# mhpi/hydrodl2

Measured on AMD Instinct MI355X. Metric: basin-ensemble-timesteps/sec fwd+bwd, higher is better.
Workload: dtype f32

## Files before the change

__graft_entry__.py:

```python
from __future__ import annotations

import os
import subprocess
import sys

ROOT = os.path.dirname(os.path.abspath(__file__))
CSRC = os.path.join(ROOT, "hydrodl2_amd", "csrc")
HIP_LIB = os.path.join(CSRC, "libhbvx.so")
ORACLE_DIR = os.path.join(ROOT, "oracle")
ORACLE_LIB = os.path.join(ORACLE_DIR, "liboracle_hbv.so")

HIPCC_FLAGS = ["--offload-arch=gfx950", "-O3", "-std=c++17", "-ffp-contract=off", "-fno-slp-vectorize", "-fPIC"]


def _newer(target: str, *sources: str) -> bool:
    if not os.path.exists(target):
        return False
    t = os.path.getmtime(target)
    return all(os.path.getmtime(s) <= t for s in sources)


def _hipcc() -> str:
    hipcc = os.environ.get("HIPCC", "/opt/rocm/bin/hipcc")
    return hipcc if os.path.exists(hipcc) else "hipcc"


def build_hip(force: bool = False, tag: str = "", flags=()) -> str:
    from concurrent.futures import ThreadPoolExecutor
    units = [os.path.join(CSRC, f) for f in sorted(os.listdir(CSRC)) if f.endswith(".hip")]
    headers = [os.path.join(CSRC, f) for f in sorted(os.listdir(CSRC)) if f.endswith(".h")] + [
        os.path.join(ROOT, "include", "hbvx.h"), os.path.join(ROOT, "include", "hbvx_lstm.h"),
        os.path.join(ROOT, "include", "hbvx_gage_pop.h")]
    objdir = os.path.join(CSRC, "build_" + tag if tag else "build")
    os.makedirs(objdir, exist_ok=True)
    extra = os.environ.get("HBVX_EXTRA_HIPCC_FLAGS", "").split() + list(flags)
    lib = os.path.join(CSRC, f"libhbvx_{tag}.so") if tag else HIP_LIB

    def compile_one(src):
        obj = os.path.join(objdir, os.path.basename(src)[:-4] + ".o")
        if force or not _newer(obj, src, *headers):
            subprocess.check_call([_hipcc()] + HIPCC_FLAGS + extra + ["-c", src, "-o", obj], cwd=CSRC)
            return obj, True
        return obj, False

    with ThreadPoolExecutor(max_workers=min(len(units), os.cpu_count() or 1)) as pool:
        done = list(pool.map(compile_one, units))
    objs = [o for o, _ in done]
    if force or any(r for _, r in done) or not _newer(lib, *objs):
        subprocess.check_call([_hipcc(), "--offload-arch=gfx950", "-shared", "-fPIC", "-o", lib] + objs, cwd=CSRC)
    return lib


def build_oracle() -> str:
    subprocess.check_call(["make", "-C", ORACLE_DIR], stdout=subprocess.DEVNULL)
    return ORACLE_LIB
# ... 57 lines not shown
```

hydrodl2_amd/_abi.py:

```python
from __future__ import annotations

import ctypes as C
import os
from typing import NamedTuple, Optional

ABI_VERSION = 10
MAX_PARAM = 20
GAGE_MAXLEN = 72
NSTATE = 5
MAX_FLUX = 12
UH_MAXLEN = 15

MODEL_HBV10, MODEL_HBV11P, MODEL_HBV20, MODEL_HBVADJ, MODEL_HOURLY = 0, 1, 2, 3, 4

TRAJ_ROWS, TRAJ_PACKED, TRAJ_CKPT = 0, 1, 2

(F_QSIM, F_Q0, F_Q1, F_Q2, F_AET, F_SWE, F_RECHARGE, F_EXCS, F_EVAPFACTOR, F_TOSOIL, F_PERC,
 F_CAPILLARY) = range(12)

PARAM_SLOTS = ["parBETA", "parFC", "parK0", "parK1", "parK2", "parLP", "parPERC", "parUZL",
               "parTT", "parCFMAX", "parCFR", "parCWH", "parBETAET", "parC", "parRT", "parAC",
               "parF0", "parFMIN", "parALPHA"]

_fp = C.c_void_p
# ... 211 lines not shown
GAGE_POP_ABI_VERSION = 1


class PopRunoff(C.Structure):
    _fields_ = [("abi_version", C.c_int32), ("n_cand", C.c_int32), ("p", PopSrc * MAX_PARAM), ("runoff", _fp)]


class GagePop(C.Structure):
    _fields_ = [("abi_version", C.c_int32), ("n_cand", C.c_int32), ("runoff", _fp), ("runoff_c_stride", C.c_int64),
                ("dp", _fp), ("uh", _fp), ("transform", C.c_int32), ("n_periods", C.c_int32),
                ("period_end", C.c_void_p),
                ("target", _fp), ("w", _fp), ("shift", _fp), ("eps", _fp),
                ("sse", _fp), ("s1", _fp), ("s2", _fp), ("s3", _fp), ("sim", _fp), ("series", _fp)]


GAGE_POP_SIGNATURES = [
    ("hbvx_gage_pop_sizeof", False, _u64, [_int], None),
    ("hbvx_hourly_population_runoff", False, _int, [_P(Desc), _P(PopRunoff), _vp], (0, PopRunoff)),
    ("hbvx_gage_population_workspace_bytes", False, _u64, [_P(GageDesc), _P(GagePop)], (1, GagePop)),
    ("hbvx_gage_population_stats", False, _int, [_P(GageDesc), _P(GagePop), _vp, _u64, _vp], (1, GagePop)),
]


class HbvxError(RuntimeError):
    pass


class Library:

    def __init__(self, path: str):
        if not os.path.exists(path):
            raise FileNotFoundError(path)
        self.path = path
        self.dll = C.CDLL(path)
        d = self.dll
        for name in EXPORTS:
            if not hasattr(d, name):
                raise HbvxError(f"{path}: missing export {name}")
        self.missing = [name for name in OPTIONAL_EXPORTS + [row[0] for row in GAGE_POP_SIGNATURES] if not hasattr(d, name)]
        checked = set()
        for name, _, restype, argtypes, layout, sizeof in [row + ("hbvx_sizeof",) for row in SIGNATURES] + \
                [row + ("hbvx_gage_pop_sizeof",) for row in GAGE_POP_SIGNATURES]:
            if name in self.missing:
                continue
            fn = getattr(d, name)
            fn.restype, fn.argtypes = restype, argtypes
            if layout is not None and (sizeof, layout[0]) not in checked and sizeof not in self.missing:
                checked.add((sizeof, layout[0]))
                which, st = layout
                got = getattr(d, sizeof)(which)
                if got != C.sizeof(st):
                    raise HbvxError(f"{path}: layout mismatch for {st.__name__}: {got} != {C.sizeof(st)}")
        if d.hbvx_version() != ABI_VERSION:
            raise HbvxError(f"{path}: ABI version {d.hbvx_version()} != {ABI_VERSION}")
        for which, st in enumerate([Desc, FwdOut, BwdIO, RouteDesc, ParamSrc, ParamGrad, GageDesc]):
            if d.hbvx_sizeof(which) != C.sizeof(st):
                raise HbvxError(f"{path}: layout mismatch for {st.__name__}: "
                                f"{d.hbvx_sizeof(which)} != {C.sizeof(st)}")
        self.backend = d.hbvx_backend().decode()
        self.saves_pow = "+savepow" in self.backend

    @property
    def is_device(self) -> bool:
        return self.backend.startswith("hip")

# ... 190 lines not shown
                                                        None if gp is None else C.byref(gp), ws, C.c_uint64(ws_bytes),
                                                        C.c_void_p(stream)), "hbvx_gage_population_stats")

    def lstm_check(self, r: LstmDesc, ws, stream: int):
        self._check(self.dll.hbvx_lstm_check(C.byref(r), ws, C.c_void_p(stream)), "hbvx_lstm_check")

    def bfi(self, T: int, B: int, qs: int, q2: int, nearzero: float, out: int, stream: int):
        self._check(self.dll.hbvx_bfi(T, B, qs, q2, C.c_float(nearzero), out, C.c_void_p(stream)),
                    "hbvx_bfi")

    def route_forward(self, r: RouteDesc, q: int, uh: int, q_rout: int, stream: int):
        self._check(self.dll.hbvx_route_forward(C.byref(r), q, uh, q_rout, C.c_void_p(stream)),
                    "hbvx_route_forward")

    def route_workspace_bytes(self, r: RouteDesc) -> int:
        return int(self.dll.hbvx_route_workspace_bytes(C.byref(r)))

    def route_backward(self, r: RouteDesc, q: int, uh: int, gqr: int, gq: int, gra, grb,
                       ws, ws_bytes: int, stream: int):
        self._check(self.dll.hbvx_route_backward(C.byref(r), q, uh, gqr, gq, gra, grb, ws,
                                                 C.c_uint64(ws_bytes), C.c_void_p(stream)),
                    "hbvx_route_backward")


def _population_method(entry: str):
    def call(self, desc, args, stream: int):
        self.require(entry)
        self._check(getattr(self.dll, entry)(None if desc is None else C.byref(desc),
                                             None if args is None else C.byref(args), C.c_void_p(stream)), entry)
    call.__name__ = entry[len("hbvx_"):]
    call.__doc__ = (f"{entry}; `desc` / `args` (its {POPULATION[entry].struct.__name__}) may be None (the ABI's own "
                    "refusals are under test).")
    return call


for _name in POPULATION:
    setattr(Library, _name[len("hbvx_"):], _population_method(_name))
```

hydrodl2_amd/csrc/hbv_chunked.h:

```cpp
#pragma once

#include <hip/hip_runtime.h>

#include "../../include/hbvx.h"
#include "hbv_step.h"
#include "hbv_lane.h"
#include "hbv_onepass_compose.h"

namespace hbvx {

struct ChunkArgs {
    hbvx_desc d;
    hbvx_bwd_io io;
    int lgMp;
    int C;
    int nchunk;
    float *phi;
    float *abnd;
    float *gpart;
    int nd;
    int dslot[3];
    int per_xcd;
    int group;
};
// ... 657 lines not shown
    const int b = (int)(n / d.M), j = (int)(n % d.M);
    if (d.raw_sigmoid) {
        const float u = sigmoid_(d.p[i].sta[(int64_t)b * d.p[i].sta_b_stride + j]);
        gsum = gsum * (u * (1.0f - u));
    }
    float *dst = io.g[i].sta + (int64_t)b * io.g[i].sta_b_stride + j;
    *dst += gsum;
}

#define ONEPASS_FOLD_GROUP 4
template <int NP>
__global__ void __launch_bounds__(256) k_bwd_chunk_fold(const ChunkArgs A)
{
    constexpr int NR = onepass_rows(NP);
    const hbvx_desc &d = A.d;
    const int64_t N = (int64_t)d.B * d.M;
    const int64_t n = (int64_t)blockIdx.x * 256 + threadIdx.x;
    if (n >= N) return;
    const int grp = blockIdx.y;
    const int c0 = grp * ONEPASS_FOLD_GROUP, c1 = min(A.nchunk, c0 + ONEPASS_FOLD_GROUP);
    double acc[NP];
#pragma unroll
    for (int i = 0; i < NP; i++) acc[i] = 0.0;
    for (int c = c0; c < c1; c++) {
        const float *g = A.gpart + (int64_t)c * NR * N + n;
        const float *ab = A.abnd + (int64_t)c * 5 * N + n;
        double a[5];
#pragma unroll
        for (int k = 0; k < 5; k++) a[k] = ab[(int64_t)k * N];
#pragma unroll
        for (int i = 0; i < NP; i++) {
            const int k0 = onepass_kmin(i), r0 = onepass_row(i);
            double v = g[(int64_t)(r0 + 5 - k0) * N];
#pragma unroll
            for (int k = 0; k < 5; k++)
                if (k >= k0) v += (double)g[(int64_t)(r0 + k - k0) * N] * a[k];
            acc[i] += v;
        }
    }
    float *dst = A.phi + (int64_t)grp * NP * N + n;
#pragma unroll
    for (int i = 0; i < NP; i++) dst[(int64_t)i * N] = (float)acc[i] * (d.p[i].hi - d.p[i].lo);
}

#endif

}
```

hydrodl2_amd/csrc/hbv_pop.h:

```cpp
#pragma once

#include <math.h>
#include <stdint.h>

#if defined(__HIPCC__)
#define HBVX_POP_HD __host__ __device__ __forceinline__
#else
#define HBVX_POP_HD inline
#endif

namespace hbvx_popk {

constexpr int UH = 15;

HBVX_POP_HD void gamma_taps(float a, float bb, int L, float (&w)[UH])
{
    float aa = fmaxf(a, 0.0f) + 0.1f;
    float theta = fmaxf(bb, 0.0f) + 0.5f;
    float denom = expf(lgammaf(aa)) * powf(theta, aa);
    float sum = 0.0f;
#pragma unroll
    for (int k = 0; k < UH; k++) {
        float t = (float)k + 0.5f;
        float mid = powf(t, aa - 1.0f);
        float right = expf(-t / theta);
        w[k] = (k < L) ? 1.0f / denom * mid * right : 0.0f;
        sum += w[k];
    }
#pragma unroll
    for (int k = 0; k < UH; k++) w[k] = (k < L) ? w[k] / sum : 0.0f;
}

struct Basin {
    float uh[UH], win[UH];
    float cost;
    bool routed;
// ... 418 lines not shown
```

hydrodl2_amd/csrc/hbvx.hip:

```cpp
#include "hbvx_host.h"
#include "hbv_step.h"
#include "hbv_lane.h"
#include "hbv_gage.h"

using namespace hbvx;
using namespace hbvx_host;

static thread_local char g_err[512] = "";

int hbvx_host::fail(int code, const char *msg)
{
    snprintf(g_err, sizeof g_err, "%s", msg);
    return code;
}

int hbvx_host::hip_fail(hipError_t e, const char *what)
{
    snprintf(g_err, sizeof g_err, "%s: %s", what, hipGetErrorString(e));
    return HBVX_E_DEVICE;
}

static std::mutex g_disp_mu;
static char g_disp[2][48] = {"", ""};
void hbvx_host::note_dispatch(int dir, const char *family)
{
    std::lock_guard<std::mutex> lock(g_disp_mu);
// ... 296 lines not shown
        for (int i = 0; i < NP; i++) {
            if (!io.g[i].sta) continue;
            float gr = raw ? gsta[i] * (usta[i] * (1.0f - usta[i])) : gsta[i];
            float *dst = io.g[i].sta + (int64_t)L.b * io.g[i].sta_b_stride + L.j;
            *dst += gr;
        }
        if (io.grad_state_in) {
#pragma unroll
            for (int k = 0; k < 5; k++) io.grad_state_in[k * N + L.n] = a[k];
        }
    }
}

__device__ __forceinline__ void route_ab(const hbvx_route_desc &r, int b, float &ua, float &ub,
                                         float &a, float &bb)
{
    float va = r.ra[(int64_t)b * r.r_stride], vb = r.rb[(int64_t)b * r.r_stride];
    ua = r.raw_sigmoid ? sigmoid_(va) : va;
    ub = r.raw_sigmoid ? sigmoid_(vb) : vb;
    a = descale_(ua, r.a_lo, r.a_hi);
    bb = descale_(ub, r.b_lo, r.b_hi);
}

__global__ void k_uh_gamma(const hbvx_route_desc r, float *__restrict__ uh)
{
    int b = blockIdx.x * blockDim.x + threadIdx.x;
    if (b >= r.B) return;
    float ua, ub, a, bb;
    route_ab(r, b, ua, ub, a, bb);
    float aa = fmaxf(a, 0.0f) + 0.1f;
    float theta = fmaxf(bb, 0.0f) + 0.5f;
    float denom = expf(lgammaf(aa)) * powf(theta, aa);
    float w[HBVX_UH_MAXLEN];
    float sum = 0.0f;
#pragma unroll
    for (int k = 0; k < HBVX_UH_MAXLEN; k++) {
        float t = (float)k + 0.5f;
        float mid = powf(t, aa - 1.0f);
        float right = expf(-t / theta);
        w[k] = (k < r.L) ? 1.0f / denom * mid * right : 0.0f;
        sum += w[k];
    }
#pragma unroll
    for (int k = 0; k < HBVX_UH_MAXLEN; k++)
        if (k < r.L) uh[(int64_t)b * r.L + k] = w[k] / sum;
}

#ifndef ROUTE_CHUNK
#define ROUTE_CHUNK 32
#endif
#ifndef ROUTE_CHUNK_BWD
#define ROUTE_CHUNK_BWD 64
#endif

__device__ __forceinline__ void load_uh(const float *__restrict__ uh, int b, int L, float *w)
{
#pragma unroll
    for (int k = 0; k < HBVX_UH_MAXLEN; k++) w[k] = (k < L) ? uh[(int64_t)b * L + k] : 0.0f;
}

#ifndef ROUTE_GROUP
#define ROUTE_GROUP 8
#endif
__global__ void __launch_bounds__(256) k_route_fwd(int T, int B, int S, int L,
                                                   const float *__restrict__ q,
                                                   const float *__restrict__ uh,
                                                   float *__restrict__ y)
{
    const int b = blockIdx.x * 64 + (threadIdx.x & 63);
    const int chunk = blockIdx.y * 4 + (threadIdx.x >> 6);
    const int t0 = chunk * ROUTE_CHUNK;
    if (b >= B || t0 >= T) return;
    const int t1 = min(T, t0 + ROUTE_CHUNK);
    const int s = blockIdx.z;
    float w[HBVX_UH_MAXLEN];
    load_uh(uh, b, L, w);
    const float *qs = q + (int64_t)s * T * B + b;
    float *ys = y + (int64_t)s * T * B + b;
    float win[HBVX_UH_MAXLEN];
#pragma unroll
    for (int k = 1; k < HBVX_UH_MAXLEN; k++) win[k] = (t0 - k >= 0) ? qs[(int64_t)(t0 - k) * B] : 0.0f;
    for (int tg = t0; tg < t1; tg += ROUTE_GROUP) {
        float v[ROUTE_GROUP];
#pragma unroll
        for (int j = 0; j < ROUTE_GROUP; j++) v[j] = (tg + j < t1) ? qs[(int64_t)(tg + j) * B] : 0.0f;
#pragma unroll
        for (int j = 0; j < ROUTE_GROUP; j++) {
            win[0] = v[j];
            float acc = 0.0f;
#pragma unroll
            for (int k = 0; k < HBVX_UH_MAXLEN; k++) acc += w[k] * win[k];
            if (tg + j < t1) ys[(int64_t)(tg + j) * B] = acc;
#pragma unroll
            for (int k = HBVX_UH_MAXLEN - 1; k > 0; k--) win[k] = win[k - 1];
        }
    }
}

__global__ void __launch_bounds__(256) k_route_bwd(int T, int B, int S, int L,
                                                   const float *__restrict__ q,
                                                   const float *__restrict__ uh,
                                                   const float *__restrict__ gy,
                                                   float *__restrict__ gq, double *__restrict__ ws)
{
    const int b = blockIdx.x * 64 + (threadIdx.x & 63);
    const int chunk = blockIdx.y * 4 + (threadIdx.x >> 6);
    const int t0 = chunk * ROUTE_CHUNK_BWD;
    if (b >= B || t0 >= T) return;
    const int t1 = min(T, t0 + ROUTE_CHUNK_BWD);
    float w[HBVX_UH_MAXLEN];
    double gw[HBVX_UH_MAXLEN];
    load_uh(uh, b, L, w);
#pragma unroll
    for (int k = 0; k < HBVX_UH_MAXLEN; k++) gw[k] = 0.0;
    for (int s = 0; s < S; s++) {
    const float *qs = q + (int64_t)s * T * B + b;
    const float *gs = gy + (int64_t)s * T * B + b;
    float *gqs = gq + (int64_t)s * T * B + b;
    float qwin[HBVX_UH_MAXLEN], gwin[HBVX_UH_MAXLEN];
#pragma unroll
    for (int k = 1; k < HBVX_UH_MAXLEN; k++) qwin[k] = (t0 - k >= 0) ? qs[(int64_t)(t0 - k) * B] : 0.0f;
#pragma unroll
    for (int k = 0; k < HBVX_UH_MAXLEN - 1; k++) gwin[k + 1] = (t0 + k < T) ? gs[(int64_t)(t0 + k) * B] : 0.0f;
    for (int tg = t0; tg < t1; tg += ROUTE_GROUP) {
        float vq[ROUTE_GROUP], vg[ROUTE_GROUP];
#pragma unroll
        for (int j = 0; j < ROUTE_GROUP; j++) {
            const int t = tg + j;
            vq[j] = (t < t1) ? qs[(int64_t)t * B] : 0.0f;
            vg[j] = (t + HBVX_UH_MAXLEN - 1 < T) ? gs[(int64_t)(t + HBVX_UH_MAXLEN - 1) * B] : 0.0f;
        }
#pragma unroll
        for (int j = 0; j < ROUTE_GROUP; j++) {
            const bool on = tg + j < t1;
#pragma unroll
            for (int k = 0; k < HBVX_UH_MAXLEN - 1; k++) gwin[k] = gwin[k + 1];
            gwin[HBVX_UH_MAXLEN - 1] = vg[j];
            qwin[0] = vq[j];
            float acc = 0.0f;
            const double g0 = on ? (double)gwin[0] : 0.0;
#pragma unroll
            for (int k = 0; k < HBVX_UH_MAXLEN; k++) {
                acc += w[k] * gwin[k];
                gw[k] = fma(g0, (double)qwin[k], gw[k]);
            }
            if (on) gqs[(int64_t)(tg + j) * B] = acc;
#pragma unroll
            for (int k = HBVX_UH_MAXLEN - 1; k > 0; k--) qwin[k] = qwin[k - 1];
        }
    }
    }
    if (ws) {
#pragma unroll
        for (int k = 0; k < HBVX_UH_MAXLEN; k++)
            if (k < L) ws[((int64_t)chunk * L + k) * B + b] = gw[k];
    }
}

__global__ void __launch_bounds__(256) k_route_tan_batch(const hbvx_route_desc r, const float *__restrict__ q,
                                                         const float *__restrict__ uh, const float *__restrict__ qd_all,
                                                         int64_t qd_ds, const float *__restrict__ rad_all,
                                                         const float *__restrict__ rbd_all, int64_t r_ds,
                                                         float *__restrict__ yd_all)
{
    const int T = r.T, B = r.B, L = r.L;
    const int b = blockIdx.x * 64 + (threadIdx.x & 63);
    const int chunk = blockIdx.y * 4 + (threadIdx.x >> 6);
    const int t0 = chunk * ROUTE_CHUNK;
    if (b >= B || t0 >= T) return;
    const int t1 = min(T, t0 + ROUTE_CHUNK);
    const int dir = blockIdx.z / r.S, s = blockIdx.z - dir * r.S;
    const float *qd = qd_all ? qd_all + dir * qd_ds : nullptr;
    const float *rad = rad_all ? rad_all + dir * r_ds : nullptr, *rbd = rbd_all ? rbd_all + dir * r_ds : nullptr;
    float *yd = yd_all + (int64_t)dir * r.S * T * B;
    float ua, ub, a, bb;
    route_ab(r, b, ua, ub, a, bb);
    const float theta = fmaxf(bb, 0.0f) + 0.5f;
    float dua = rad ? rad[(int64_t)b * r.r_stride] : 0.0f, dub = rbd ? rbd[(int64_t)b * r.r_stride] : 0.0f;
// ... 38 lines not shown
        for (int k = HBVX_UH_MAXLEN - 1; k > 0; k--) {
            win[k] = win[k - 1];
            dwin[k] = dwin[k - 1];
        }
    }
}

#define ROUTE_PB 16
__global__ void __launch_bounds__(1024) k_route_bwd_params(const hbvx_route_desc r, int nchunk,
                                                           const float *__restrict__ uh,
                                                           const double *__restrict__ ws,
                                                           float *grad_ra, float *grad_rb)
{
    __shared__ double prt[4][16][ROUTE_PB];
    __shared__ double red[16][ROUTE_PB];
    const int bl = threadIdx.x & (ROUTE_PB - 1), k = (threadIdx.x >> 4) & 15, part = threadIdx.x >> 8;
    const int b = blockIdx.x * ROUTE_PB + bl;
    const int B = r.B, L = r.L;
    double acc = 0.0;
    if (b < B && k < L) {
        const double *src = ws + (int64_t)k * B + b;
        const int64_t cs = (int64_t)L * B;
        const int n4 = nchunk & ~3;
        for (int c = part; c < n4; c += 4) acc += src[(int64_t)c * cs];
        if (part == 0)
            for (int c = n4; c < nchunk; c++) acc += src[(int64_t)c * cs];
    }
    prt[part][k][bl] = acc;
    __syncthreads();
    if (part == 0) red[k][bl] = (prt[0][k][bl] + prt[1][k][bl]) + (prt[2][k][bl] + prt[3][k][bl]);
    __syncthreads();
    if (part != 0 || k != 0 || b >= B) return;
    float ua, ub, a, bb;
    route_ab(r, b, ua, ub, a, bb);
    const float theta = fmaxf(bb, 0.0f) + 0.5f;
    double w[HBVX_UH_MAXLEN], gw[HBVX_UH_MAXLEN];
    double mlt = 0.0, mt = 0.0;
#pragma unroll
    for (int j = 0; j < HBVX_UH_MAXLEN; j++) {
        gw[j] = (j < L) ? red[j][bl] : 0.0;
        w[j] = (j < L) ? (double)uh[(int64_t)b * L + j] : 0.0;
        const double tk = (double)j + 0.5;
        mlt += w[j] * log(tk);
        mt += w[j] * tk;
    }
    double gaa = 0.0, gth = 0.0;
    const double th2 = (double)theta * (double)theta;
// ... 212 lines not shown
    });
    if (e != hipSuccess) return hip_fail(e, "hbvx_backward launch");
    return HBVX_OK;
}

static int check_route(const hbvx_route_desc *r)
{
    if (!r) return fail(HBVX_E_NULL, "route desc is NULL");
    if (r->abi_version != HBVX_ABI_VERSION) return fail(HBVX_E_ABI, "abi_version mismatch");
    if (r->T <= 0 || r->B <= 0 || r->S <= 0) return fail(HBVX_E_SHAPE, "bad T/B/S");
    const int L = r->T < HBVX_UH_MAXLEN ? r->T : HBVX_UH_MAXLEN;
    if (r->L != L) return fail(HBVX_E_SHAPE, "L must be min(T, 15)");
    if (!r->ra || !r->rb) return fail(HBVX_E_NULL, "routing parameter pointer is NULL");
    return HBVX_OK;
}

extern "C" int hbvx_route_forward(const hbvx_route_desc *r, const float *q, float *uh,
                                  float *q_rout, void *stream)
{
    int rc = check_route(r);
    if (rc) return rc;
    if (!q || !uh || !q_rout) return fail(HBVX_E_NULL, "route buffer is NULL");
    hipStream_t st = (hipStream_t)stream;
    hipLaunchKernelGGL(k_uh_gamma, dim3((r->B + 63) / 64), dim3(64), 0, st, *r, uh);
    const int nchunk = (r->T + ROUTE_CHUNK - 1) / ROUTE_CHUNK;
    hipLaunchKernelGGL(k_route_fwd, dim3((r->B + 63) / 64, (nchunk + 3) / 4, r->S), dim3(256), 0, st, r->T,
                       r->B, r->S, r->L, q, uh, q_rout);
    hipError_t e = hipGetLastError();
    if (e != hipSuccess) return hip_fail(e, "hbvx_route_forward launch");
    return HBVX_OK;
}

static int route_chunks(const hbvx_route_desc *r) { return (r->T + ROUTE_CHUNK_BWD - 1) / ROUTE_CHUNK_BWD; }

extern "C" uint64_t hbvx_route_workspace_bytes(const hbvx_route_desc *r)
{
    if (!r || r->T <= 0 || r->B <= 0) return 0;
    return (uint64_t)route_chunks(r) * (uint64_t)r->L * (uint64_t)r->B * sizeof(double);
}

extern "C" int hbvx_route_backward(const hbvx_route_desc *r, const float *q, const float *uh,
                                   const float *grad_q_rout, float *grad_q, float *grad_ra,
                                   float *grad_rb, void *workspace, uint64_t workspace_bytes,
                                   void *stream)
{
    int rc = check_route(r);
    if (rc) return rc;
    if (!q || !uh || !grad_q_rout || !grad_q) return fail(HBVX_E_NULL, "route buffer is NULL");
    hipStream_t st = (hipStream_t)stream;
    const bool want_p = grad_ra || grad_rb;
    if (want_p && (!workspace || workspace_bytes < hbvx_route_workspace_bytes(r)))
        return fail(HBVX_E_NULL, "route workspace missing or too small");
    const int nchunk = route_chunks(r);
    hipLaunchKernelGGL(k_route_bwd, dim3((r->B + 63) / 64, (nchunk + 3) / 4), dim3(256), 0, st, r->T,
                       r->B, r->S, r->L, q, uh, grad_q_rout, grad_q, want_p ? (double *)workspace : nullptr);
    if (want_p)
        hipLaunchKernelGGL(k_route_bwd_params, dim3((r->B + ROUTE_PB - 1) / ROUTE_PB), dim3(1024), 0, st, *r, nchunk,
                           uh, (const double *)workspace, grad_ra, grad_rb);
    hipError_t e = hipGetLastError();
    if (e != hipSuccess) return hip_fail(e, "hbvx_route_backward launch");
    return HBVX_OK;
}

__global__ void k_selftest_pow(const float *x, const float *y, float *out, int n)
{
    int i = blockIdx.x * blockDim.x + threadIdx.x;
    if (i < n) out[i] = pow_pos_(x[i], y[i]);
}

extern "C" int hbvx_selftest_pow(const float *x, const float *y, float *out, int n, void *stream)
{
    if (!x || !y || !out || n <= 0) return fail(HBVX_E_NULL, "selftest_pow: bad arguments");
    hipLaunchKernelGGL(k_selftest_pow, dim3((n + 255) / 256), dim3(256), 0, (hipStream_t)stream, x, y,
                       out, n);
    hipError_t e = hipGetLastError();
    if (e != hipSuccess) return hip_fail(e, "selftest_pow launch");
    return HBVX_OK;
}

__global__ void k_selftest_div(const float *x, const float *y, float *out, int n)
{
    int i = blockIdx.x * blockDim.x + threadIdx.x;
    if (i < n) out[i] = div_(x[i], y[i]);
}

extern "C" int hbvx_selftest_div(const float *x, const float *y, float *out, int n, void *stream)
{
    if (!x || !y || !out || n <= 0) return fail(HBVX_E_NULL, "selftest_div: bad arguments");
    hipLaunchKernelGGL(k_selftest_div, dim3((n + 255) / 256), dim3(256), 0, (hipStream_t)stream, x, y,
                       out, n);
    hipError_t e = hipGetLastError();
    if (e != hipSuccess) return hip_fail(e, "selftest_div launch");
    return HBVX_OK;
}

__global__ void __launch_bounds__(1024) k_bfi(int T, int B, const float *__restrict__ qs,
                                              const float *__restrict__ q2, float nz,
                                              float *__restrict__ bfi)
{
    __shared__ float r0[64][16], r2[64][16];
    const int bl = threadIdx.x & 15, sl = threadIdx.x >> 4;
    const int b = blockIdx.x * 16 + bl;
    float a0 = 0.0f, a2 = 0.0f, c0 = 0.0f, c2 = 0.0f;
    if (b < B) {
        int t = sl;
        for (; t + 64 < T; t += 128) {
            a0 += qs[(int64_t)t * B + b];
            a2 += q2[(int64_t)t * B + b];
            c0 += qs[(int64_t)(t + 64) * B + b];
            c2 += q2[(int64_t)(t + 64) * B + b];
        }
        if (t < T) {
            a0 += qs[(int64_t)t * B + b];
            a2 += q2[(int64_t)t * B + b];
        }
    }
    r0[sl][bl] = a0 + c0;
    r2[sl][bl] = a2 + c2;
    __syncthreads();
    if (sl == 0 && b < B) {
        float s0 = 0.0f, s2 = 0.0f;
#pragma unroll
        for (int k = 0; k < 64; k++) {
            s0 += r0[k][bl];
            s2 += r2[k][bl];
        }
        bfi[b] = 100.0f * (s2 / (s0 + nz));
    }
}

extern "C" int hbvx_bfi(int32_t T, int32_t B, const float *qs, const float *q2, float nearzero,
                        float *bfi, void *stream)
{
    if (!qs || !q2 || !bfi || T <= 0 || B <= 0) return fail(HBVX_E_NULL, "hbvx_bfi: bad arguments");
    hipLaunchKernelGGL(k_bfi, dim3((B + 15) / 16), dim3(1024), 0, (hipStream_t)stream, T, B, qs, q2,
                       nearzero, bfi);
    hipError_t e = hipGetLastError();
    if (e != hipSuccess) return hip_fail(e, "hbvx_bfi launch");
    return HBVX_OK;
}

__device__ __forceinline__ void bfi_tan_body(int T, int B, const float *__restrict__ qs,
                                             const float *__restrict__ q2, const float *__restrict__ qsd,
                                             const float *__restrict__ q2d, float nz, float *__restrict__ bfid)
{
    __shared__ float r0[64][16], r2[64][16], d0[64][16], d2[64][16];
    const int bl = threadIdx.x & 15, sl = threadIdx.x >> 4;
    const int b = blockIdx.x * 16 + bl;
    float a0 = 0.0f, a2 = 0.0f, e0 = 0.0f, e2 = 0.0f;
    if (b < B) {
        for (int t = sl; t < T; t += 64) {
            a0 += qs[(int64_t)t * B + b];
            a2 += q2[(int64_t)t * B + b];
            e0 += qsd ? qsd[(int64_t)t * B + b] : 0.0f;
            e2 += q2d ? q2d[(int64_t)t * B + b] : 0.0f;
        }
    }
    r0[sl][bl] = a0;
    r2[sl][bl] = a2;
// ... 351 lines not shown
```

hydrodl2_amd/ops.py:

```python
from __future__ import annotations

import contextlib
import ctypes as _C
from dataclasses import dataclass, field
import functools
import os
import struct
import threading
from typing import List, NamedTuple, Optional, Sequence

import torch
import torch.autograd.forward_ad as _fwAD

from . import _abi
from ._lib import get_library


@dataclass
class ParamSource:
    slot: int
    lo: float
    hi: float
    tensor_idx: int
    sta_off: int
# ... 543 lines not shown
        if _FILL_OVERLAP and lib.is_device:
            gp, rows, bases, start_fill = _overlapped_grad_buffers(lib, cfg, ptensors, ctx.needs_input_grad[6:], early)
        else:
            gp = [_grad_like(lib, p, cfg, i) if ctx.needs_input_grad[6 + i] else None
                  for i, p in enumerate(ptensors)]

        def sta_ptr(idx, off):
            return _ptr(rows[idx], off - bases[idx]) if rows[idx] is not None else _ptr(gp[idx], off)

        def join():
            nonlocal fill_done
            if start_fill is not None and fill_done is None:
                fill_done = start_fill()
            if fill_done is not None:
                torch.cuda.current_stream(dev).wait_event(fill_done)
            for big, row in zip(gp, rows):
                if row is not None:
                    big[-1] += row

        gq = None
        if g_routed is not None and cfg.route is not None:
            r = _route_desc(cfg, ptensors, S=n_live)
            gq = _out((4, T, B), dev)
            if n_live < 4:
                gq[n_live:].zero_()
            rs = cfg.route
            gt = gp[rs.tensor_idx]
            ws_bytes = _cached(cfg, ("route_ws", n_live), lambda: lib.route_workspace_bytes(r))
            ws = torch.empty((max(ws_bytes, 4) + 3) // 4, dtype=torch.float32, device=dev)
            g_routed = g_routed.contiguous()
            _call(lib, 'hbvx_route_backward', lib.route_backward, r, _ptr(flux), _ptr(uh),
                  _ptr(g_routed), _ptr(gq), sta_ptr(rs.tensor_idx, rs.a_off) if gt is not None else None,
                  sta_ptr(rs.tensor_idx, rs.b_off) if gt is not None else None,
                  _ptr(ws), ws_bytes, stream)
        have = [k for k, g in enumerate(g_rows) if g is not None]
        g_flux = None
        if have and max(have) < 4:
            if gq is None:
                gq = torch.zeros((4, T, B), dtype=torch.float32, device=dev)
            for k in have:
                gq[k] += g_rows[k]
        elif have:
            g_flux = torch.zeros((cfg.n_flux, T, B), dtype=torch.float32, device=dev)
            for k in have:
                g_flux[k] = g_rows[k]

        io = _abi.BwdIO()
        io.traj, io.aux = _ptr(traj), _ptr(aux)
        io.grad_flux, io.grad_flux4 = _ptr(g_flux), _ptr(gq)
        io.n_flux, io.traj_layout = cfg.n_flux, ctx.traj_layout
        gx = gmu = None
        if ctx.needs_input_grad[1]:
            gx = _zeros_like(lib, x)
            if gx.stride() != x.stride():
                raise ValueError("x_phy must be dense for a forcing gradient")
            io.grad_x = _ptr(gx, cfg.t0 * x.stride(0))
        if muwts is not None and ctx.needs_input_grad[3]:
# ... 861 lines not shown
```

Baseline: 34.55 billion.

## Stage routing windows in LDS, swizzle blocks across XCDs, fuse gradient zeroing

The routing forward and backward kernels now stage the q and gradient windows in shared memory and split taps and days across the four waves. Blocks are remapped so that consecutive tiles land on the same XCD. A new rows entry point zeroes the unused gq rows inside the backward launch instead of using a separate fill. Separately, the gamma unit hydrograph is computed with one thread per tap, the BFI reduction gets wider unrolled variants with XCD swizzling, and the onepass fold loads two chunks at a time. Together these aim to cut redundant global loads and launch overhead, at the cost of more shared memory per block and more code paths.

Result: faster. 35.94 billion, median of 6 (+4.0%).

```diff
diff --git a/__graft_entry__.py b/__graft_entry__.py
--- a/__graft_entry__.py
+++ b/__graft_entry__.py
@@ -30,7 +30,7 @@
     units = [os.path.join(CSRC, f) for f in sorted(os.listdir(CSRC)) if f.endswith(".hip")]
     headers = [os.path.join(CSRC, f) for f in sorted(os.listdir(CSRC)) if f.endswith(".h")] + [
         os.path.join(ROOT, "include", "hbvx.h"), os.path.join(ROOT, "include", "hbvx_lstm.h"),
-        os.path.join(ROOT, "include", "hbvx_gage_pop.h")]
+        os.path.join(ROOT, "include", "hbvx_gage_pop.h"), os.path.join(ROOT, "include", "hbvx_route_rows.h")]
     objdir = os.path.join(CSRC, "build_" + tag if tag else "build")
     os.makedirs(objdir, exist_ok=True)
     extra = os.environ.get("HBVX_EXTRA_HIPCC_FLAGS", "").split() + list(flags)
diff --git a/hydrodl2_amd/_abi.py b/hydrodl2_amd/_abi.py
--- a/hydrodl2_amd/_abi.py
+++ b/hydrodl2_amd/_abi.py
@@ -257,6 +257,11 @@
 ]
 
 
+ROUTE_ROWS_SIGNATURES = [
+    ("hbvx_route_backward_rows", False, _int, [_P(RouteDesc), _fp, _fp, _fp, _fp, _i32, _fp, _fp, _fp, _u64, _vp], None),
+]
+
+
 class HbvxError(RuntimeError):
     pass
 
@@ -272,10 +277,12 @@
         for name in EXPORTS:
             if not hasattr(d, name):
                 raise HbvxError(f"{path}: missing export {name}")
-        self.missing = [name for name in OPTIONAL_EXPORTS + [row[0] for row in GAGE_POP_SIGNATURES] if not hasattr(d, name)]
+        self.missing = [name for name in OPTIONAL_EXPORTS + [row[0] for row in GAGE_POP_SIGNATURES + ROUTE_ROWS_SIGNATURES]
+                        if not hasattr(d, name)]
         checked = set()
         for name, _, restype, argtypes, layout, sizeof in [row + ("hbvx_sizeof",) for row in SIGNATURES] + \
-                [row + ("hbvx_gage_pop_sizeof",) for row in GAGE_POP_SIGNATURES]:
+                [row + ("hbvx_gage_pop_sizeof",) for row in GAGE_POP_SIGNATURES] + \
+                [row + ("hbvx_sizeof",) for row in ROUTE_ROWS_SIGNATURES]:
             if name in self.missing:
                 continue
             fn = getattr(d, name)
@@ -512,6 +519,13 @@
                                                  C.c_uint64(ws_bytes), C.c_void_p(stream)),
                     "hbvx_route_backward")
 
+    def route_backward_rows(self, r: RouteDesc, q: int, uh: int, gqr: int, gq: int, gq_rows: int, gra, grb,
+                            ws, ws_bytes: int, stream: int):
+        self.require("hbvx_route_backward_rows")
+        self._check(self.dll.hbvx_route_backward_rows(C.byref(r), q, uh, gqr, gq, gq_rows, gra, grb, ws,
+                                                      C.c_uint64(ws_bytes), C.c_void_p(stream)),
+                    "hbvx_route_backward_rows")
+
 
 def _population_method(entry: str):
     def call(self, desc, args, stream: int):
diff --git a/hydrodl2_amd/csrc/hbv_chunked.h b/hydrodl2_amd/csrc/hbv_chunked.h
--- a/hydrodl2_amd/csrc/hbv_chunked.h
+++ b/hydrodl2_amd/csrc/hbv_chunked.h
@@ -703,21 +703,40 @@
     double acc[NP];
 #pragma unroll
     for (int i = 0; i < NP; i++) acc[i] = 0.0;
-    for (int c = c0; c < c1; c++) {
+    auto load = [&](int c, float (&gv)[NR], float (&av)[5]) {
         const float *g = A.gpart + (int64_t)c * NR * N + n;
         const float *ab = A.abnd + (int64_t)c * 5 * N + n;
+#pragma unroll
+        for (int k = 0; k < 5; k++) av[k] = ab[(int64_t)k * N];
+#pragma unroll
+        for (int r = 0; r < NR; r++) gv[r] = g[(int64_t)r * N];
+    };
+    auto fold = [&](const float (&gv)[NR], const float (&av)[5]) {
         double a[5];
 #pragma unroll
-        for (int k = 0; k < 5; k++) a[k] = ab[(int64_t)k * N];
+        for (int k = 0; k < 5; k++) a[k] = av[k];
 #pragma unroll
         for (int i = 0; i < NP; i++) {
             const int k0 = onepass_kmin(i), r0 = onepass_row(i);
-            double v = g[(int64_t)(r0 + 5 - k0) * N];
+            double v = gv[r0 + 5 - k0];
 #pragma unroll
             for (int k = 0; k < 5; k++)
-                if (k >= k0) v += (double)g[(int64_t)(r0 + k - k0) * N] * a[k];
+                if (k >= k0) v += (double)gv[r0 + k - k0] * a[k];
             acc[i] += v;
         }
+    };
+    int c = c0;
+    for (; c + 1 < c1; c += 2) {
+        float g0[NR], a0[5], g1[NR], a1[5];
+        load(c, g0, a0);
+        load(c + 1, g1, a1);
+        fold(g0, a0);
+        fold(g1, a1);
+    }
+    if (c < c1) {
+        float g0[NR], a0[5];
+        load(c, g0, a0);
+        fold(g0, a0);
     }
     float *dst = A.phi + (int64_t)grp * NP * N + n;
 #pragma unroll
diff --git a/hydrodl2_amd/csrc/hbv_pop.h b/hydrodl2_amd/csrc/hbv_pop.h
--- a/hydrodl2_amd/csrc/hbv_pop.h
+++ b/hydrodl2_amd/csrc/hbv_pop.h
@@ -12,6 +12,15 @@
 namespace hbvx_popk {
 
 constexpr int UH = 15;
+
+HBVX_POP_HD float gamma_denom(float aa, float theta) { return expf(lgammaf(aa)) * powf(theta, aa); }
+HBVX_POP_HD float gamma_tap(float denom, float aa, float theta, int k)
+{
+    float t = (float)k + 0.5f;
+    float mid = powf(t, aa - 1.0f);
+    float right = expf(-t / theta);
+    return 1.0f / denom * mid * right;
+}
 
 HBVX_POP_HD void gamma_taps(float a, float bb, int L, float (&w)[UH])
 {
diff --git a/hydrodl2_amd/csrc/hbvx.hip b/hydrodl2_amd/csrc/hbvx.hip
--- a/hydrodl2_amd/csrc/hbvx.hip
+++ b/hydrodl2_amd/csrc/hbvx.hip
@@ -1,7 +1,9 @@
 #include "hbvx_host.h"
+#include "../../include/hbvx_route_rows.h"
 #include "hbv_step.h"
 #include "hbv_lane.h"
 #include "hbv_gage.h"
+#include "hbv_pop.h"
 
 using namespace hbvx;
 using namespace hbvx_host;
@@ -344,28 +346,29 @@
     bb = descale_(ub, r.b_lo, r.b_hi);
 }
 
-__global__ void k_uh_gamma(const hbvx_route_desc r, float *__restrict__ uh)
-{
-    int b = blockIdx.x * blockDim.x + threadIdx.x;
-    if (b >= r.B) return;
-    float ua, ub, a, bb;
-    route_ab(r, b, ua, ub, a, bb);
-    float aa = fmaxf(a, 0.0f) + 0.1f;
-    float theta = fmaxf(bb, 0.0f) + 0.5f;
-    float denom = expf(lgammaf(aa)) * powf(theta, aa);
-    float w[HBVX_UH_MAXLEN];
+#define UH_PB 16
+__global__ void __launch_bounds__(16 * UH_PB) k_uh_gamma(const hbvx_route_desc r, float *__restrict__ uh)
+{
+    static_assert(HBVX_UH_MAXLEN <= 16, "k_uh_gamma: 16 tap slots");
+    __shared__ float sw[16][UH_PB];
+    const int bl = threadIdx.x % UH_PB, k = threadIdx.x / UH_PB;
+    const int b = blockIdx.x * UH_PB + bl;
+    const bool mine = b < r.B && k < r.L;
+    float v = 0.0f;
+    if (mine) {
+        float ua, ub, a, bb;
+        route_ab(r, b, ua, ub, a, bb);
+        float aa = fmaxf(a, 0.0f) + 0.1f;
+        float theta = fmaxf(bb, 0.0f) + 0.5f;
+        v = hbvx_popk::gamma_tap(hbvx_popk::gamma_denom(aa, theta), aa, theta, k);
+    }
+    sw[k][bl] = v;
+    __syncthreads();
+    if (!mine) return;
     float sum = 0.0f;
 #pragma unroll
-    for (int k = 0; k < HBVX_UH_MAXLEN; k++) {
-        float t = (float)k + 0.5f;
-        float mid = powf(t, aa - 1.0f);
-        float right = expf(-t / theta);
-        w[k] = (k < r.L) ? 1.0f / denom * mid * right : 0.0f;
-        sum += w[k];
-    }
-#pragma unroll
-    for (int k = 0; k < HBVX_UH_MAXLEN; k++)
-        if (k < r.L) uh[(int64_t)b * r.L + k] = w[k] / sum;
+    for (int j = 0; j < HBVX_UH_MAXLEN; j++) sum += sw[j][bl];
+    uh[(int64_t)b * r.L + k] = v / sum;
 }
 
 #ifndef ROUTE_CHUNK
@@ -375,107 +378,154 @@
 #define ROUTE_CHUNK_BWD 64
 #endif
 
+static inline unsigned xcd_grid(int64_t n) { return (unsigned)((n + 7) / 8 * 8); }
+__device__ __forceinline__ int xcd_block()
+{
+    const int per = gridDim.x / 8;
+    return (blockIdx.x % 8) * per + blockIdx.x / 8;
+}
+
 __device__ __forceinline__ void load_uh(const float *__restrict__ uh, int b, int L, float *w)
 {
 #pragma unroll
     for (int k = 0; k < HBVX_UH_MAXLEN; k++) w[k] = (k < L) ? uh[(int64_t)b * L + k] : 0.0f;
 }
 
-#ifndef ROUTE_GROUP
-#define ROUTE_GROUP 8
-#endif
+#define ROUTE_FWD_TILE (4 * ROUTE_CHUNK)
+#define ROUTE_FWD_ROWS (ROUTE_FWD_TILE + HBVX_UH_MAXLEN - 1)
 __global__ void __launch_bounds__(256) k_route_fwd(int T, int B, int S, int L,
                                                    const float *__restrict__ q,
                                                    const float *__restrict__ uh,
                                                    float *__restrict__ y)
 {
-    const int b = blockIdx.x * 64 + (threadIdx.x & 63);
-    const int chunk = blockIdx.y * 4 + (threadIdx.x >> 6);
-    const int t0 = chunk * ROUTE_CHUNK;
-    if (b >= B || t0 >= T) return;
-    const int t1 = min(T, t0 + ROUTE_CHUNK);
-    const int s = blockIdx.z;
+    __shared__ float sq[ROUTE_FWD_ROWS][64];
+    constexpr int NLOAD = (ROUTE_FWD_ROWS + 3) / 4;
+    const int lane = threadIdx.x & 63, part = __builtin_amdgcn_readfirstlane(threadIdx.x >> 6);
+    const int nx = (B + 63) / 64, ny = (T + ROUTE_FWD_TILE - 1) / ROUTE_FWD_TILE;
+    const int blk = xcd_block();
+    if (blk >= nx * ny * S) return;
+    const int b = (blk % nx) * 64 + lane;
+    const int t0 = (blk / nx) % ny * ROUTE_FWD_TILE;
+    const bool live = b < B;
+    const int s = blk / (nx * ny);
+    const float *qs = q + (int64_t)s * T * B;
+    float *ys = y + (int64_t)s * T * B;
+    float v[NLOAD];
+#pragma unroll
+    for (int i = 0; i < NLOAD; i++) {
+        const int r = part + 4 * i, t = t0 - (HBVX_UH_MAXLEN - 1) + r;
+        v[i] = (live && r < ROUTE_FWD_ROWS && t >= 0 && t < T) ? (qs + (int64_t)t * B)[b] : 0.0f;
+    }
     float w[HBVX_UH_MAXLEN];
-    load_uh(uh, b, L, w);
-    const float *qs = q + (int64_t)s * T * B + b;
-    float *ys = y + (int64_t)s * T * B + b;
+    load_uh(uh, live ? b : B - 1, L, w);
+#pragma unroll
+    for (int i = 0; i < NLOAD; i++) {
+        const int r = part + 4 * i;
+        if (r < ROUTE_FWD_ROWS) sq[r][lane] = v[i];
+    }
+    __syncthreads();
+    const int c0 = part * ROUTE_CHUNK;
+    if (!live || t0 + c0 >= T) return;
     float win[HBVX_UH_MAXLEN];
 #pragma unroll
-    for (int k = 1; k < HBVX_UH_MAXLEN; k++) win[k] = (t0 - k >= 0) ? qs[(int64_t)(t0 - k) * B] : 0.0f;
-    for (int tg = t0; tg < t1; tg += ROUTE_GROUP) {
-        float v[ROUTE_GROUP];
-#pragma unroll
-        for (int j = 0; j < ROUTE_GROUP; j++) v[j] = (tg + j < t1) ? qs[(int64_t)(tg + j) * B] : 0.0f;
-#pragma unroll
-        for (int j = 0; j < ROUTE_GROUP; j++) {
-            win[0] = v[j];
-            float acc = 0.0f;
-#pragma unroll
-            for (int k = 0; k < HBVX_UH_MAXLEN; k++) acc += w[k] * win[k];
-            if (tg + j < t1) ys[(int64_t)(tg + j) * B] = acc;
-#pragma unroll
-            for (int k = HBVX_UH_MAXLEN - 1; k > 0; k--) win[k] = win[k - 1];
-        }
-    }
-}
-
-__global__ void __launch_bounds__(256) k_route_bwd(int T, int B, int S, int L,
+    for (int k = 1; k < HBVX_UH_MAXLEN; k++) win[k] = sq[c0 + HBVX_UH_MAXLEN - 1 - k][lane];
+#pragma unroll 8
+    for (int d = 0; d < ROUTE_CHUNK; d++) {
+        win[0] = sq[c0 + HBVX_UH_MAXLEN - 1 + d][lane];
+        float acc = 0.0f;
+#pragma unroll
+        for (int k = 0; k < HBVX_UH_MAXLEN; k++) acc += w[k] * win[k];
+        if (t0 + c0 + d < T) (ys + (int64_t)(t0 + c0 + d) * B)[b] = acc;
+#pragma unroll
+        for (int k = HBVX_UH_MAXLEN - 1; k > 0; k--) win[k] = win[k - 1];
+    }
+}
+
+#define ROUTE_BWD_ROWS (ROUTE_CHUNK_BWD + HBVX_UH_MAXLEN - 1)
+#define ROUTE_BWD_DAYS (ROUTE_CHUNK_BWD / 4)
+#define ROUTE_BWD_TAPS 4
+static_assert(ROUTE_CHUNK_BWD % 4 == 0 && 4 * ROUTE_BWD_TAPS >= HBVX_UH_MAXLEN, "k_route_bwd: four waves share a chunk");
+__global__ void __launch_bounds__(256) k_route_bwd(int T, int B, int S, int L, int n_rows,
                                                    const float *__restrict__ q,
                                                    const float *__restrict__ uh,
                                                    const float *__restrict__ gy,
                                                    float *__restrict__ gq, double *__restrict__ ws)
 {
-    const int b = blockIdx.x * 64 + (threadIdx.x & 63);
-    const int chunk = blockIdx.y * 4 + (threadIdx.x >> 6);
+    __shared__ float sq[ROUTE_BWD_ROWS][64], sg[ROUTE_BWD_ROWS][64];
+    constexpr int NLOAD = (ROUTE_BWD_ROWS + 3) / 4;
+    const int lane = threadIdx.x & 63, part = __builtin_amdgcn_readfirstlane(threadIdx.x >> 6);
+    const int nx = (B + 63) / 64;
+    const int blk = xcd_block();
+    if (blk >= nx * ((T + ROUTE_CHUNK_BWD - 1) / ROUTE_CHUNK_BWD)) return;
+    const int b = (blk % nx) * 64 + lane;
+    const int chunk = blk / nx;
     const int t0 = chunk * ROUTE_CHUNK_BWD;
-    if (b >= B || t0 >= T) return;
     const int t1 = min(T, t0 + ROUTE_CHUNK_BWD);
+    const bool live = b < B;
+    const int d0 = part * ROUTE_BWD_DAYS, k0 = part * ROUTE_BWD_TAPS;
     float w[HBVX_UH_MAXLEN];
-    double gw[HBVX_UH_MAXLEN];
-    load_uh(uh, b, L, w);
-#pragma unroll
-    for (int k = 0; k < HBVX_UH_MAXLEN; k++) gw[k] = 0.0;
+    double gw[ROUTE_BWD_TAPS];
+    load_uh(uh, live ? b : B - 1, L, w);
+#pragma unroll
+    for (int j = 0; j < ROUTE_BWD_TAPS; j++) gw[j] = 0.0;
     for (int s = 0; s < S; s++) {
-    const float *qs = q + (int64_t)s * T * B + b;
-    const float *gs = gy + (int64_t)s * T * B + b;
-    float *gqs = gq + (int64_t)s * T * B + b;
-    float qwin[HBVX_UH_MAXLEN], gwin[HBVX_UH_MAXLEN];
-#pragma unroll
-    for (int k = 1; k < HBVX_UH_MAXLEN; k++) qwin[k] = (t0 - k >= 0) ? qs[(int64_t)(t0 - k) * B] : 0.0f;
-#pragma unroll
-    for (int k = 0; k < HBVX_UH_MAXLEN - 1; k++) gwin[k + 1] = (t0 + k < T) ? gs[(int64_t)(t0 + k) * B] : 0.0f;
-    for (int tg = t0; tg < t1; tg += ROUTE_GROUP) {
-        float vq[ROUTE_GROUP], vg[ROUTE_GROUP];
-#pragma unroll
-        for (int j = 0; j < ROUTE_GROUP; j++) {
-            const int t = tg + j;
-            vq[j] = (t < t1) ? qs[(int64_t)t * B] : 0.0f;
-            vg[j] = (t + HBVX_UH_MAXLEN - 1 < T) ? gs[(int64_t)(t + HBVX_UH_MAXLEN - 1) * B] : 0.0f;
-        }
-#pragma unroll
-        for (int j = 0; j < ROUTE_GROUP; j++) {
-            const bool on = tg + j < t1;
-#pragma unroll
-            for (int k = 0; k < HBVX_UH_MAXLEN - 1; k++) gwin[k] = gwin[k + 1];
-            gwin[HBVX_UH_MAXLEN - 1] = vg[j];
-            qwin[0] = vq[j];
+        const float *qs = q + (int64_t)s * T * B;
+        const float *gs = gy + (int64_t)s * T * B;
+        float *gqs = gq + (int64_t)s * T * B;
+        float vq[NLOAD], vg[NLOAD];
+#pragma unroll
+        for (int i = 0; i < NLOAD; i++) {
+            const int r = part + 4 * i, tq = t0 - (HBVX_UH_MAXLEN - 1) + r, tg = t0 + r;
+            const bool in = live && r < ROUTE_BWD_ROWS;
+            vq[i] = (in && tq >= 0 && tq < t1) ? (qs + (int64_t)tq * B)[b] : 0.0f;
+            vg[i] = (in && tg < T) ? (gs + (int64_t)tg * B)[b] : 0.0f;
+        }
+        if (s) __syncthreads();
+#pragma unroll
+        for (int i = 0; i < NLOAD; i++) {
+            const int r = part + 4 * i;
+            if (r < ROUTE_BWD_ROWS) {
+                sq[r][lane] = vq[i];
+                sg[r][lane] = vg[i];
+            }
+        }
+        __syncthreads();
+        if (s == 0 && live) {
+            for (int z = S; z < n_rows; z++) {
+                float *gz = gq + (int64_t)z * T * B;
+#pragma unroll
+                for (int d = 0; d < ROUTE_BWD_DAYS; d++)
+                    if (t0 + d0 + d < t1) (gz + (int64_t)(t0 + d0 + d) * B)[b] = 0.0f;
+            }
+        }
+        float g[ROUTE_BWD_DAYS + HBVX_UH_MAXLEN - 1];
+#pragma unroll
+        for (int i = 0; i < ROUTE_BWD_DAYS + HBVX_UH_MAXLEN - 1; i++) g[i] = sg[d0 + i][lane];
+#pragma unroll
+        for (int d = 0; d < ROUTE_BWD_DAYS; d++) {
             float acc = 0.0f;
-            const double g0 = on ? (double)gwin[0] : 0.0;
-#pragma unroll
-            for (int k = 0; k < HBVX_UH_MAXLEN; k++) {
-                acc += w[k] * gwin[k];
-                gw[k] = fma(g0, (double)qwin[k], gw[k]);
-            }
-            if (on) gqs[(int64_t)(tg + j) * B] = acc;
-#pragma unroll
-            for (int k = HBVX_UH_MAXLEN - 1; k > 0; k--) qwin[k] = qwin[k - 1];
-        }
-    }
-    }
-    if (ws) {
-#pragma unroll
-        for (int k = 0; k < HBVX_UH_MAXLEN; k++)
-            if (k < L) ws[((int64_t)chunk * L + k) * B + b] = gw[k];
+#pragma unroll
+            for (int k = 0; k < HBVX_UH_MAXLEN; k++) acc += w[k] * g[d + k];
+            if (live && t0 + d0 + d < t1) (gqs + (int64_t)(t0 + d0 + d) * B)[b] = acc;
+        }
+        double qw[ROUTE_BWD_TAPS];
+#pragma unroll
+        for (int j = 1; j < ROUTE_BWD_TAPS; j++) qw[j] = (double)sq[max(HBVX_UH_MAXLEN - 1 - k0 - j, 0)][lane];
+        const int nd = t1 - t0;
+#pragma unroll 8
+        for (int i = 0; i < nd; i++) {
+            qw[0] = (double)sq[i + HBVX_UH_MAXLEN - 1 - k0][lane];
+            const double g0 = (double)sg[i][lane];
+#pragma unroll
+            for (int j = 0; j < ROUTE_BWD_TAPS; j++) gw[j] = fma(g0, qw[j], gw[j]);
+#pragma unroll
+            for (int j = ROUTE_BWD_TAPS - 1; j > 0; j--) qw[j] = qw[j - 1];
+        }
+    }
+    if (ws && live) {
+#pragma unroll
+        for (int j = 0; j < ROUTE_BWD_TAPS; j++)
+            if (k0 + j < L) ws[((int64_t)chunk * L + k0 + j) * B + b] = gw[j];
     }
 }
 
@@ -560,7 +610,15 @@
         const double *src = ws + (int64_t)k * B + b;
         const int64_t cs = (int64_t)L * B;
         const int n4 = nchunk & ~3;
-        for (int c = part; c < n4; c += 4) acc += src[(int64_t)c * cs];
+        int c = part;
+        for (; c + 4 * 7 < n4; c += 4 * 8) {
+            double v[8];
+#pragma unroll
+            for (int j = 0; j < 8; j++) v[j] = src[(int64_t)(c + 4 * j) * cs];
+#pragma unroll
+            for (int j = 0; j < 8; j++) acc += v[j];
+        }
+        for (; c < n4; c += 4) acc += src[(int64_t)c * cs];
         if (part == 0)
             for (int c = n4; c < nchunk; c++) acc += src[(int64_t)c * cs];
     }
@@ -819,10 +877,10 @@
     if (rc) return rc;
     if (!q || !uh || !q_rout) return fail(HBVX_E_NULL, "route buffer is NULL");
     hipStream_t st = (hipStream_t)stream;
-    hipLaunchKernelGGL(k_uh_gamma, dim3((r->B + 63) / 64), dim3(64), 0, st, *r, uh);
-    const int nchunk = (r->T + ROUTE_CHUNK - 1) / ROUTE_CHUNK;
-    hipLaunchKernelGGL(k_route_fwd, dim3((r->B + 63) / 64, (nchunk + 3) / 4, r->S), dim3(256), 0, st, r->T,
-                       r->B, r->S, r->L, q, uh, q_rout);
+    hipLaunchKernelGGL(k_uh_gamma, dim3((r->B + UH_PB - 1) / UH_PB), dim3(16 * UH_PB), 0, st, *r, uh);
+    const int64_t nblk = (int64_t)((r->B + 63) / 64) * ((r->T + ROUTE_FWD_TILE - 1) / ROUTE_FWD_TILE) * r->S;
+    if (nblk > INT32_MAX - 8) return fail(HBVX_E_SHAPE, "routing: too many (basin, day, series) tiles for one launch");
+    hipLaunchKernelGGL(k_route_fwd, dim3(xcd_grid(nblk)), dim3(256), 0, st, r->T, r->B, r->S, r->L, q, uh, q_rout);
     hipError_t e = hipGetLastError();
     if (e != hipSuccess) return hip_fail(e, "hbvx_route_forward launch");
     return HBVX_OK;
@@ -836,27 +894,46 @@
     return (uint64_t)route_chunks(r) * (uint64_t)r->L * (uint64_t)r->B * sizeof(double);
 }
 
-extern "C" int hbvx_route_backward(const hbvx_route_desc *r, const float *q, const float *uh,
-                                   const float *grad_q_rout, float *grad_q, float *grad_ra,
-                                   float *grad_rb, void *workspace, uint64_t workspace_bytes,
-                                   void *stream)
+static int launch_route_bwd(const hbvx_route_desc *r, const float *q, const float *uh, const float *grad_q_rout,
+                            float *grad_q, int n_rows, float *grad_ra, float *grad_rb, void *workspace,
+                            uint64_t workspace_bytes, void *stream, const char *what)
 {
     int rc = check_route(r);
     if (rc) return rc;
     if (!q || !uh || !grad_q_rout || !grad_q) return fail(HBVX_E_NULL, "route buffer is NULL");
+    if (n_rows < r->S) return fail(HBVX_E_SHAPE, "grad_q has fewer rows than series");
     hipStream_t st = (hipStream_t)stream;
     const bool want_p = grad_ra || grad_rb;
     if (want_p && (!workspace || workspace_bytes < hbvx_route_workspace_bytes(r)))
         return fail(HBVX_E_NULL, "route workspace missing or too small");
     const int nchunk = route_chunks(r);
-    hipLaunchKernelGGL(k_route_bwd, dim3((r->B + 63) / 64, (nchunk + 3) / 4), dim3(256), 0, st, r->T,
-                       r->B, r->S, r->L, q, uh, grad_q_rout, grad_q, want_p ? (double *)workspace : nullptr);
+    const int64_t nblk = (int64_t)((r->B + 63) / 64) * nchunk;
+    if (nblk > INT32_MAX - 8) return fail(HBVX_E_SHAPE, "routing adjoint: too many (basin, chunk) tiles for one launch");
+    hipLaunchKernelGGL(k_route_bwd, dim3(xcd_grid(nblk)), dim3(256), 0, st, r->T, r->B, r->S, r->L, n_rows, q, uh,
+                       grad_q_rout, grad_q, want_p ? (double *)workspace : nullptr);
     if (want_p)
         hipLaunchKernelGGL(k_route_bwd_params, dim3((r->B + ROUTE_PB - 1) / ROUTE_PB), dim3(1024), 0, st, *r, nchunk,
                            uh, (const double *)workspace, grad_ra, grad_rb);
     hipError_t e = hipGetLastError();
-    if (e != hipSuccess) return hip_fail(e, "hbvx_route_backward launch");
+    if (e != hipSuccess) return hip_fail(e, what);
     return HBVX_OK;
+}
+
+extern "C" int hbvx_route_backward(const hbvx_route_desc *r, const float *q, const float *uh,
+                                   const float *grad_q_rout, float *grad_q, float *grad_ra,
+                                   float *grad_rb, void *workspace, uint64_t workspace_bytes,
+                                   void *stream)
+{
+    return launch_route_bwd(r, q, uh, grad_q_rout, grad_q, r ? r->S : 0, grad_ra, grad_rb, workspace, workspace_bytes,
+                            stream, "hbvx_route_backward launch");
+}
+
+extern "C" int hbvx_route_backward_rows(const hbvx_route_desc *r, const float *q, const float *uh,
+                                        const float *grad_q_rout, float *grad_q, int32_t grad_q_rows, float *grad_ra,
+                                        float *grad_rb, void *workspace, uint64_t workspace_bytes, void *stream)
+{
+    return launch_route_bwd(r, q, uh, grad_q_rout, grad_q, grad_q_rows, grad_ra, grad_rb, workspace, workspace_bytes,
+                            stream, "hbvx_route_backward_rows launch");
 }
 
 __global__ void k_selftest_pow(const float *x, const float *y, float *out, int n)
@@ -891,47 +968,74 @@
     return HBVX_OK;
 }
 
-__global__ void __launch_bounds__(1024) k_bfi(int T, int B, const float *__restrict__ qs,
-                                              const float *__restrict__ q2, float nz,
-                                              float *__restrict__ bfi)
-{
-    __shared__ float r0[64][16], r2[64][16];
-    const int bl = threadIdx.x & 15, sl = threadIdx.x >> 4;
-    const int b = blockIdx.x * 16 + bl;
-    float a0 = 0.0f, a2 = 0.0f, c0 = 0.0f, c2 = 0.0f;
+#define BFI_ROWS 8
+template <int PB, int NH>
+__global__ void __launch_bounds__(PB * 64 * NH) k_bfi(int T, int B, const float *__restrict__ qs,
+                                                      const float *__restrict__ q2, float nz,
+                                                      float *__restrict__ bfi)
+{
+    constexpr int NC = 2 / NH, NR = BFI_ROWS / NC;
+    __shared__ float r0[2][64][PB], r2[2][64][PB];
+    const int bl = threadIdx.x % PB, sl = (threadIdx.x / PB) & 63, half = threadIdx.x / (PB * 64);
+    const int b = xcd_block() * PB + bl;
+    float a0[NC], a2[NC];
+#pragma unroll
+    for (int i = 0; i < NC; i++) a0[i] = a2[i] = 0.0f;
     if (b < B) {
+        const int h0 = half * NC;
         int t = sl;
-        for (; t + 64 < T; t += 128) {
-            a0 += qs[(int64_t)t * B + b];
-            a2 += q2[(int64_t)t * B + b];
-            c0 += qs[(int64_t)(t + 64) * B + b];
-            c2 += q2[(int64_t)(t + 64) * B + b];
-        }
-        if (t < T) {
-            a0 += qs[(int64_t)t * B + b];
-            a2 += q2[(int64_t)t * B + b];
-        }
-    }
-    r0[sl][bl] = a0 + c0;
-    r2[sl][bl] = a2 + c2;
+        for (; t + 64 * (h0 + NC - 1) + 128 * (NR - 1) < T; t += 128 * NR) {
+            float v0[NC][NR], v2[NC][NR];
+#pragma unroll
+            for (int j = 0; j < NR; j++)
+#pragma unroll
+                for (int i = 0; i < NC; i++) {
+                    v0[i][j] = qs[(int64_t)(t + 64 * (h0 + i) + 128 * j) * B + b];
+                    v2[i][j] = q2[(int64_t)(t + 64 * (h0 + i) + 128 * j) * B + b];
+                }
+#pragma unroll
+            for (int j = 0; j < NR; j++)
+#pragma unroll
+                for (int i = 0; i < NC; i++) {
+                    a0[i] += v0[i][j];
+                    a2[i] += v2[i][j];
+                }
+        }
+#pragma unroll
+        for (int i = 0; i < NC; i++)
+            for (int tt = t + 64 * (h0 + i); tt < T; tt += 128) {
+                a0[i] += qs[(int64_t)tt * B + b];
+                a2[i] += q2[(int64_t)tt * B + b];
+            }
+    }
+#pragma unroll
+    for (int i = 0; i < NC; i++) {
+        r0[half * NC + i][sl][bl] = a0[i];
+        r2[half * NC + i][sl][bl] = a2[i];
+    }
     __syncthreads();
-    if (sl == 0 && b < B) {
+    if (threadIdx.x < PB && b < B) {
         float s0 = 0.0f, s2 = 0.0f;
 #pragma unroll
         for (int k = 0; k < 64; k++) {
-            s0 += r0[k][bl];
-            s2 += r2[k][bl];
+            s0 += r0[0][k][bl] + r0[1][k][bl];
+            s2 += r2[0][k][bl] + r2[1][k][bl];
         }
         bfi[b] = 100.0f * (s2 / (s0 + nz));
     }
 }
 
+#define BFI_WIDE_BLOCKS 256
 extern "C" int hbvx_bfi(int32_t T, int32_t B, const float *qs, const float *q2, float nearzero,
                         float *bfi, void *stream)
 {
     if (!qs || !q2 || !bfi || T <= 0 || B <= 0) return fail(HBVX_E_NULL, "hbvx_bfi: bad arguments");
-    hipLaunchKernelGGL(k_bfi, dim3((B + 15) / 16), dim3(1024), 0, (hipStream_t)stream, T, B, qs, q2,
-                       nearzero, bfi);
+    if ((B + 15) / 16 >= BFI_WIDE_BLOCKS)
+        hipLaunchKernelGGL((k_bfi<16, 1>), dim3(xcd_grid((B + 15) / 16)), dim3(1024), 0, (hipStream_t)stream, T, B, qs, q2,
+                           nearzero, bfi);
+    else
+        hipLaunchKernelGGL((k_bfi<4, 2>), dim3(xcd_grid((B + 3) / 4)), dim3(512), 0, (hipStream_t)stream, T, B, qs, q2,
+                           nearzero, bfi);
     hipError_t e = hipGetLastError();
     if (e != hipSuccess) return hip_fail(e, "hbvx_bfi launch");
     return HBVX_OK;
diff --git a/hydrodl2_amd/ops.py b/hydrodl2_amd/ops.py
--- a/hydrodl2_amd/ops.py
+++ b/hydrodl2_amd/ops.py
@@ -589,17 +589,22 @@
         if g_routed is not None and cfg.route is not None:
             r = _route_desc(cfg, ptensors, S=n_live)
             gq = _out((4, T, B), dev)
-            if n_live < 4:
+            in_launch = n_live < 4 and "hbvx_route_backward_rows" not in lib.missing
+            if n_live < 4 and not in_launch:
                 gq[n_live:].zero_()
             rs = cfg.route
             gt = gp[rs.tensor_idx]
             ws_bytes = _cached(cfg, ("route_ws", n_live), lambda: lib.route_workspace_bytes(r))
             ws = torch.empty((max(ws_bytes, 4) + 3) // 4, dtype=torch.float32, device=dev)
             g_routed = g_routed.contiguous()
-            _call(lib, 'hbvx_route_backward', lib.route_backward, r, _ptr(flux), _ptr(uh),
-                  _ptr(g_routed), _ptr(gq), sta_ptr(rs.tensor_idx, rs.a_off) if gt is not None else None,
-                  sta_ptr(rs.tensor_idx, rs.b_off) if gt is not None else None,
-                  _ptr(ws), ws_bytes, stream)
+            g_ab = (sta_ptr(rs.tensor_idx, rs.a_off) if gt is not None else None,
+                    sta_ptr(rs.tensor_idx, rs.b_off) if gt is not None else None)
+            if in_launch:
+                _call(lib, 'hbvx_route_backward', lib.route_backward_rows, r, _ptr(flux), _ptr(uh),
+                      _ptr(g_routed), _ptr(gq), 4, *g_ab, _ptr(ws), ws_bytes, stream)
+            else:
+                _call(lib, 'hbvx_route_backward', lib.route_backward, r, _ptr(flux), _ptr(uh),
+                      _ptr(g_routed), _ptr(gq), *g_ab, _ptr(ws), ws_bytes, stream)
         have = [k for k, g in enumerate(g_rows) if g is not None]
         g_flux = None
         if have and max(have) < 4:
diff --git a/include/hbvx_route_rows.h b/include/hbvx_route_rows.h
--- /dev/null
+++ b/include/hbvx_route_rows.h
@@ -0,0 +1,18 @@
+#ifndef HBVX_ROUTE_ROWS_H
+#define HBVX_ROUTE_ROWS_H
+
+#include "hbvx.h"
+
+#ifdef __cplusplus
+extern "C" {
+#endif
+
+int hbvx_route_backward_rows(const hbvx_route_desc *r, const float *q, const float *uh,
+                             const float *grad_q_rout, float *grad_q, int32_t grad_q_rows, float *grad_ra,
+                             float *grad_rb, void *workspace, uint64_t workspace_bytes, void *stream);
+
+#ifdef __cplusplus
+}
+#endif
+
+#endif
```
